# KAIST-VICLab/MoBGS

Measured on AMD Instinct MI355X. Metric: train-step renders/sec (fwd+bwd, 1352x1014, 300k Gaussians), higher is better.
Workload: dtype f32; 1 GPU; BASELINE config #2: seesaw-synth (SURVEY 8d seed 0), 200000 static + 100000 dynamic Gaussians, 1352x1014, render() lean mode fwd+bwd incl. spline prep, decoder, camera gradient; gaussians=300000, visible=287203, pixels=1370928, parallelism=single

## Files before the change

### mobgs_amd/csrc/decoder_shared.h

```cpp
#pragma once
#include "common.h"
#include "wave_shared.h"

namespace mobgs {

constexpr int W1_ROWS_SHARED = 2;

typedef const float __attribute__((address_space(4))) * ConstWeights;
__device__ __forceinline__ ConstWeights reload_here(const float* p) {
    unsigned long long v = (unsigned long long)p;
    asm volatile("" : "+s"(v));
    const unsigned lo = __builtin_amdgcn_readfirstlane((unsigned)v);
    const unsigned hi = __builtin_amdgcn_readfirstlane((unsigned)(v >> 32));
    return (ConstWeights)(((unsigned long long)hi << 32) | lo);
}

struct RayCam {
    float fx, fy, cx, cy;
    float c2w[12];
};
__device__ inline RayCam load_raycam(const float* __restrict__ intr, const float* __restrict__ c2w) {
    RayCam c;
    c.fx = intr[0]; c.fy = intr[1]; c.cx = intr[2]; c.cy = intr[3];
#pragma unroll
// ... 140 lines not shown
    vf[9] = g / ac;
    v_alpha = alpha > 1e-10f ? -g * f[9] / (ac * ac) : 0.f;
#pragma unroll
    for (int i = 0; i < 3; ++i) {
        vorg[i] = vx[6 + i];
        vdir[i] = vx[9 + i];
    }
}

struct WgradFinish {
    const float* w_partial = nullptr;
    float *g_w1 = nullptr, *g_w2 = nullptr, *g_c2w = nullptr;
    int rows_per_image = 0, n_images = 0, accumulate = 0, c2w_floats = 0;
};
constexpr int WGRAD_NRED = 102;
__host__ __device__ inline int wgrad_finish_outputs(const WgradFinish& f) {
    return WGRAD_NRED + ((f.g_c2w && f.c2w_floats == 16) ? 4 : 0);
}
__device__ inline void wgrad_column_sum(const WgradFinish& f, int k, int img) {
    float* g_c2w = f.g_c2w ? f.g_c2w + (size_t)img * f.c2w_floats : nullptr;
    if (k >= WGRAD_NRED) {
        if (threadIdx.x == 0) g_c2w[k - 90] = 0.f;
        return;
    }
    int first = 0, count = f.rows_per_image * f.n_images;
    if (k >= 90) {
        first = img * f.rows_per_image;
        count = f.rows_per_image;
    } else if (img != 0) {
        return;
    }
    const float* wp = f.w_partial + (size_t)first * WGRAD_NRED;
    float s = 0.f;
    for (int b = threadIdx.x; b < count; b += 256) s += wp[(size_t)b * WGRAD_NRED + k];
    MOBGS_WAVE_FOLD(s, MOBGS_WAVE_ADD);
    __shared__ float wgrad_red[4];
    if ((threadIdx.x & 63) == 0) wgrad_red[threadIdx.x >> 6] = s;
    __syncthreads();
    if (threadIdx.x == 0) {
        const float t = wgrad_red[0] + wgrad_red[1] + wgrad_red[2] + wgrad_red[3];
        if (k < 72)
            f.g_w1[k] = f.accumulate ? f.g_w1[k] + t : t;
        else if (k < 90)
            f.g_w2[k - 72] = f.accumulate ? f.g_w2[k - 72] + t : t;
        else if (g_c2w)
            g_c2w[k - 90] = t;
    }
}

size_t decoder_wgrad_scratch_floats(int C, int rows_per_image);
unsigned* decoder_wgrad_ticket(float* scratch, int C, int rows_per_image);
void launch_decoder_wgrad_reduce(int C, int rows_per_image, float* scratch, float* g_w1, float* g_w2, float* g_c2w,
                                 int g_c2w_floats, int accumulate, hipStream_t st);

}
```

### mobgs_amd/csrc/prep_shared.h

```cpp
#pragma once
#include <hip/hip_fp16.h>

#include "common.h"

namespace mobgs {

__device__ inline float ldf(const float* p, size_t i) { return p[i]; }
__device__ inline float ldf(const __half* p, size_t i) { return __half2float(p[i]); }
__device__ inline float4 ld4(const float* p, size_t i) { return reinterpret_cast<const float4*>(p)[i]; }
__device__ inline float4 ld4(const __half* p, size_t i) {
    const uint2 u = reinterpret_cast<const uint2*>(p)[i];
    const __half2 a = *reinterpret_cast<const __half2*>(&u.x), b = *reinterpret_cast<const __half2*>(&u.y);
    const float2 fa = __half22float2(a), fb = __half22float2(b);
    return make_float4(fa.x, fa.y, fb.x, fb.y);
}
__device__ inline void stf(float* p, size_t i, float v) { p[i] = v; }
__device__ inline void stf(__half* p, size_t i, float v) { p[i] = __float2half(v); }
__device__ inline void st4(float* p, size_t i, float4 v) { reinterpret_cast<float4*>(p)[i] = v; }
__device__ inline void st4(__half* p, size_t i, float4 v) {
    const __half2 a = __floats2half2_rn(v.x, v.y), b = __floats2half2_rn(v.z, v.w);
    uint2 u;
    u.x = *reinterpret_cast<const unsigned*>(&a);
    u.y = *reinterpret_cast<const unsigned*>(&b);
    reinterpret_cast<uint2*>(p)[i] = u;
// ... 58 lines not shown
            s[k] = expf(ldf(in.s_scaling, 3 * (size_t)i + k));
            col[6 + k] = 0.0f * ldf(in.s_ft, 3 * (size_t)i + k);
        }
        const float4 r = ld4(in.s_rotation, i);
        q[0] = r.x; q[1] = r.y; q[2] = r.z; q[3] = r.w;
        o = 1.f / (1.f + expf(-ldf(in.s_opacity, i)));
#pragma unroll
        for (int k = 0; k < 6; ++k) col[k] = ldf(in.s_fdc, 6 * (size_t)i + k);
    } else {
        const int j = i - in.Ns;
        const float t_feat = in.times[0], t_curve = in.times[1];
        const float tfp = t_feat - in.d_trbf[j];
        const int n = (int)in.d_ncp[j];
        const Hermite H = hermite_setup(t_curve, n);
        const float* cp = in.d_control + (size_t)j * 36;
#pragma unroll
        for (int k = 0; k < 3; ++k) {
            const float p0 = cp[3 * H.i0 + k], p1 = cp[3 * H.i1 + k], p2 = cp[3 * H.i2 + k], p3 = cp[3 * H.i3 + k];
            const float m0 = H.left_edge ? (p2 - p1) : (p2 - p0) * 0.5f;
            const float m1 = H.right_edge ? (p2 - p1) : (p3 - p1) * 0.5f;
            m[k] = (H.h00 * p1 + H.h10 * m0 + H.h01 * p2 + H.h11 * m1) * 1e-2f;
            s[k] = expf(ldf(in.d_scaling, 3 * (size_t)j + k));
            col[6 + k] = tfp * ldf(in.d_ft, 3 * (size_t)j + k);
        }
        const float4 r = ld4(in.d_rotation, j);
        const float4 w = ld4(in.d_omega, j);
        q[0] = r.x + tfp * w.x; q[1] = r.y + tfp * w.y; q[2] = r.z + tfp * w.z; q[3] = r.w + tfp * w.w;
        o = 1.f / (1.f + expf(-ldf(in.d_opacity, j)));
#pragma unroll
        for (int k = 0; k < 6; ++k) col[k] = ldf(in.d_fdc, 6 * (size_t)j + k);
    }
}

template <bool ACC, typename G>
__device__ __forceinline__ void prep_bwd_apply(
    int i, int Ns, const float* __restrict__ times, const long long* __restrict__ d_ncp,
    const float* __restrict__ d_trbf, const float (&vm)[3], const float (&vq)[4], const float (&vs)[3], float vo,
    const float (&vc)[9], float* __restrict__ g_s_xyz, G* __restrict__ g_s_scaling, G* __restrict__ g_s_rotation,
    G* __restrict__ g_s_opacity, G* __restrict__ g_s_fdc, G* __restrict__ g_s_ft, float* __restrict__ g_d_control,
    G* __restrict__ g_d_scaling, G* __restrict__ g_d_rotation, G* __restrict__ g_d_omega, G* __restrict__ g_d_opacity,
    G* __restrict__ g_d_fdc, G* __restrict__ g_d_ft) {
#pragma clang fp contract(off)
    if (i < Ns) {
#pragma unroll
        for (int k = 0; k < 3; ++k) {
            g_s_xyz[3 * i + k] = (ACC ? g_s_xyz[3 * i + k] : 0.f) + vm[k];
            stf(g_s_scaling, 3 * (size_t)i + k, (ACC ? ldf(g_s_scaling, 3 * (size_t)i + k) : 0.f) + vs[k]);
            stf(g_s_ft, 3 * (size_t)i + k, (ACC ? ldf(g_s_ft, 3 * (size_t)i + k) : 0.f) + 0.0f * vc[6 + k]);
        }
        {
            float4 q = make_float4(vq[0], vq[1], vq[2], vq[3]);
            if (ACC) {
                const float4 o = ld4(g_s_rotation, i);
                q = make_float4(o.x + q.x, o.y + q.y, o.z + q.z, o.w + q.w);
            }
            st4(g_s_rotation, i, q);
        }
        stf(g_s_opacity, i, (ACC ? ldf(g_s_opacity, i) : 0.f) + vo);
#pragma unroll
        for (int k = 0; k < 6; ++k) stf(g_s_fdc, 6 * (size_t)i + k, (ACC ? ldf(g_s_fdc, 6 * (size_t)i + k) : 0.f) + vc[k]);
    } else {
        const int j = i - Ns;
        const float tfp = times[0] - d_trbf[j];
        const int n = (int)d_ncp[j];
        const Hermite H = hermite_setup(times[1], n);
        float* gc = g_d_control + (size_t)j * 36;
#pragma unroll
        for (int k = 0; k < 3; ++k) {
            const float v = vm[k] * 1e-2f;
            float a0 = 0.f, a1 = H.h00 * v, a2 = H.h01 * v, a3 = 0.f;
            const float vm0 = H.h10 * v, vm1 = H.h11 * v;
            if (H.left_edge) {
                a2 += vm0;
                a1 -= vm0;
            } else {
                a2 += 0.5f * vm0;
                a0 -= 0.5f * vm0;
            }
            if (H.right_edge) {
                a2 += vm1;
                a1 -= vm1;
            } else {
                a3 += 0.5f * vm1;
                a1 -= 0.5f * vm1;
            }
            if (ACC) {
                if (!H.left_edge) gc[3 * H.i0 + k] += a0;
                gc[3 * H.i1 + k] += a1;
                gc[3 * H.i2 + k] += a2;
                if (!H.right_edge) gc[3 * H.i3 + k] += a3;
            } else {
                if (!H.left_edge) gc[3 * H.i0 + k] = a0;
                gc[3 * H.i1 + k] = a1;
                gc[3 * H.i2 + k] = a2;
                if (!H.right_edge) gc[3 * H.i3 + k] = a3;
            }
            stf(g_d_scaling, 3 * (size_t)j + k, (ACC ? ldf(g_d_scaling, 3 * (size_t)j + k) : 0.f) + vs[k]);
            stf(g_d_ft, 3 * (size_t)j + k, (ACC ? ldf(g_d_ft, 3 * (size_t)j + k) : 0.f) + tfp * vc[6 + k]);
        }
        {
            float4 q = make_float4(vq[0], vq[1], vq[2], vq[3]);
            float4 w = make_float4(tfp * vq[0], tfp * vq[1], tfp * vq[2], tfp * vq[3]);
            if (ACC) {
                const float4 o = ld4(g_d_rotation, j);
                const float4 p = ld4(g_d_omega, j);
                q = make_float4(o.x + q.x, o.y + q.y, o.z + q.z, o.w + q.w);
                w = make_float4(p.x + w.x, p.y + w.y, p.z + w.z, p.w + w.w);
            }
            st4(g_d_rotation, j, q);
            st4(g_d_omega, j, w);
        }
        stf(g_d_opacity, j, (ACC ? ldf(g_d_opacity, j) : 0.f) + vo);
#pragma unroll
        for (int k = 0; k < 6; ++k) stf(g_d_fdc, 6 * (size_t)j + k, (ACC ? ldf(g_d_fdc, 6 * (size_t)j + k) : 0.f) + vc[k]);
    }
}

__device__ __forceinline__ void prep_bwd_clear_rows(int Ns, int Nd, float* __restrict__ g_d_control) {
    const int wave_first = (blockIdx.x * blockDim.x + (threadIdx.x & ~63)) - Ns;
    const int j0 = max(wave_first, 0), j1 = min(wave_first + 64, Nd);
    if (j1 > j0) {
        float4* row = reinterpret_cast<float4*>(g_d_control + (size_t)j0 * 36);
        const int n4 = (j1 - j0) * 9;
        for (int t = threadIdx.x & 63; t < n4; t += 64) row[t] = make_float4(0.f, 0.f, 0.f, 0.f);
        __builtin_amdgcn_fence(__ATOMIC_RELEASE, "wavefront");
        __builtin_amdgcn_s_waitcnt(0);
    }
}

}
```

### mobgs_amd/csrc/project.hip

```cpp
#include <stdarg.h>

#include "isect_launch.h"
#include "prep_shared.h"
#include "wave_shared.h"

namespace mobgs {

static thread_local char g_err[512] = "";
void set_error(const char* fmt, ...) {
    va_list ap;
    va_start(ap, fmt);
    vsnprintf(g_err, sizeof(g_err), fmt, ap);
    va_end(ap);
}

struct Cam {
    float R[9];
    float t[3];
    float fx, fy, cx, cy;
};

__device__ inline Cam load_cam(const float* __restrict__ viewmats, const float* __restrict__ Ks, int c) {
    Cam cam;
    const float* V = viewmats + 16 * c;
// ... 214 lines not shown
struct PrepBwdFused {
    int Ns, Nd, accumulate;
    const float* times;
    const long long* d_ncp;
    const float *d_trbf, *opac, *v_opac, *v_colors;
    const float *x_means, *x_quats, *x_scales;
    LeafGrads g;
};
template <bool PREPB>
__global__ void __launch_bounds__(256)
project_bwd_kernel(int N, const float* __restrict__ means, const float* __restrict__ quats,
                   const float* __restrict__ scales, const float* __restrict__ viewmats,
                   const float* __restrict__ Ks, int width, int height, float eps2d,
                   const int32_t* __restrict__ radii, const float* __restrict__ conics,
                   const float* __restrict__ v_means2d, const float* __restrict__ v_depths,
                   const float* __restrict__ v_conics, float* __restrict__ v_means,
                   float* __restrict__ v_quats, float* __restrict__ v_scales,
                   float* __restrict__ v_view_partial, int accumulate, int accumulate_scales, size_t geom_stride,
                   size_t scales_stride, PrepBwdFused pb) {
    const int i = blockIdx.x * blockDim.x + threadIdx.x;
    const int c = blockIdx.y;
    if constexpr (PREPB) {
        if (!pb.accumulate) prep_bwd_clear_rows(pb.Ns, pb.Nd, pb.g.d_control);
    }
    means += 3 * c * geom_stride;
    quats += 4 * c * geom_stride;
    v_means += 3 * c * geom_stride;
    v_quats += 4 * c * geom_stride;
    v_scales += 3 * c * scales_stride;
    const Cam cam = load_cam(viewmats, Ks, c);
    float vR[9] = {0.f, 0.f, 0.f, 0.f, 0.f, 0.f, 0.f, 0.f, 0.f};
    float vt[3] = {0.f, 0.f, 0.f};
    float vm[3] = {0.f, 0.f, 0.f}, vq[4] = {0.f, 0.f, 0.f, 0.f}, vs[3] = {0.f, 0.f, 0.f};
    const size_t o = (size_t)c * N + (i < N ? i : 0);
    const bool live = (i < N) && radii[o] > 0;
    if (live) {
        const float m[3] = {means[3 * i], means[3 * i + 1], means[3 * i + 2]};
        float p[3];
#pragma unroll
        for (int r = 0; r < 3; ++r)
            p[r] = cam.R[3 * r] * m[0] + cam.R[3 * r + 1] * m[1] + cam.R[3 * r + 2] * m[2] + cam.t[r];
        const float4 qv = reinterpret_cast<const float4*>(quats)[i];
        const float qraw[4] = {qv.x, qv.y, qv.z, qv.w};
        const float s[3] = {scales[3 * i], scales[3 * i + 1], scales[3 * i + 2]};
        float Rq[9], M[9], S3[9], RS[9], Sc[9];
        quat_to_rotmat(qraw, Rq);
#pragma unroll
        for (int r = 0; r < 3; ++r) {
            M[3 * r] = Rq[3 * r] * s[0];
            M[3 * r + 1] = Rq[3 * r + 1] * s[1];
            M[3 * r + 2] = Rq[3 * r + 2] * s[2];
        }
        mm3_abt(M, M, S3);
        mm3(cam.R, S3, RS);
        mm3_abt(RS, cam.R, Sc);
        const Persp P = persp_setup(cam, p, width, height);

        const float X0 = conics[3 * o], X1 = conics[3 * o + 1], X2 = conics[3 * o + 2];
        float g0 = 0.f, g1 = 0.f, g2 = 0.f;
        if (v_conics) {
            g0 = v_conics[3 * o];
            g1 = 0.5f * v_conics[3 * o + 1];
            g2 = v_conics[3 * o + 2];
        }
        const float A00 = X0 * g0 + X1 * g1, A01 = X0 * g1 + X1 * g2;
        const float A10 = X1 * g0 + X2 * g1, A11 = X1 * g1 + X2 * g2;
        const float vS00 = -(A00 * X0 + A01 * X1), vS01 = -(A00 * X1 + A01 * X2);
        const float vS10 = -(A10 * X0 + A11 * X1), vS11 = -(A10 * X1 + A11 * X2);

        float vSJ[6];
#pragma unroll
        for (int k = 0; k < 3; ++k) {
            vSJ[k] = vS00 * P.J[k] + vS01 * P.J[3 + k];
            vSJ[3 + k] = vS10 * P.J[k] + vS11 * P.J[3 + k];
        }
        float vSc[9];
#pragma unroll
        for (int a = 0; a < 3; ++a)
#pragma unroll
            for (int b = 0; b < 3; ++b) vSc[3 * a + b] = P.J[a] * vSJ[b] + P.J[3 + a] * vSJ[3 + b];
        float vStJ[6];
#pragma unroll
        for (int k = 0; k < 3; ++k) {
            vStJ[k] = vS00 * P.J[k] + vS10 * P.J[3 + k];
            vStJ[3 + k] = vS01 * P.J[k] + vS11 * P.J[3 + k];
        }
        float vJ[6];
#pragma unroll
        for (int r = 0; r < 2; ++r)
#pragma unroll
            for (int k = 0; k < 3; ++k) {
                vJ[3 * r + k] = vSJ[3 * r] * Sc[3 * k] + vSJ[3 * r + 1] * Sc[3 * k + 1] + vSJ[3 * r + 2] * Sc[3 * k + 2] +
                                vStJ[3 * r] * Sc[k] + vStJ[3 * r + 1] * Sc[3 + k] + vStJ[3 * r + 2] * Sc[6 + k];
            }

        float vp[3] = {0.f, 0.f, 0.f};
        float gx = 0.f, gy = 0.f;
        if (v_means2d) {
            gx = v_means2d[2 * o];
            gy = v_means2d[2 * o + 1];
        }
        const float rz = P.rz, rz2 = P.rz2, rz3 = rz2 * rz;
        vp[0] += cam.fx * rz * gx;
        vp[1] += cam.fy * rz * gy;
        vp[2] += -(cam.fx * p[0] * gx + cam.fy * p[1] * gy) * rz2;
        const float xr = p[0] * rz, yr = p[1] * rz;
        if (xr <= P.lim_x_pos && xr >= -P.lim_x_neg)
            vp[0] += -cam.fx * rz2 * vJ[2];
        else
            vp[2] += -cam.fx * rz3 * vJ[2] * P.tx;
        if (yr <= P.lim_y_pos && yr >= -P.lim_y_neg)
            vp[1] += -cam.fy * rz2 * vJ[5];
        else
            vp[2] += -cam.fy * rz3 * vJ[5] * P.ty;
        vp[2] += -cam.fx * rz2 * vJ[0] - cam.fy * rz2 * vJ[4] + 2.f * cam.fx * P.tx * rz3 * vJ[2] +
                 2.f * cam.fy * P.ty * rz3 * vJ[5];
        if (v_depths) vp[2] += v_depths[o];

#pragma unroll
        for (int r = 0; r < 3; ++r) {
            vt[r] = vp[r];
#pragma unroll
            for (int k = 0; k < 3; ++k) vR[3 * r + k] = vp[r] * m[k];
        }
#pragma unroll
        for (int k = 0; k < 3; ++k) vm[k] = cam.R[k] * vp[0] + cam.R[3 + k] * vp[1] + cam.R[6 + k] * vp[2];

        float RS3t[9];
        mm3_abt(cam.R, S3, RS3t);
        float T1[9], T2[9];
        mm3(vSc, RS3t, T1);
        mm3_atb(vSc, RS, T2);
#pragma unroll
        for (int k = 0; k < 9; ++k) vR[k] += T1[k] + T2[k];
        float RtV[9], vS3[9];
        mm3_atb(cam.R, vSc, RtV);
        mm3(RtV, cam.R, vS3);

        float Sy[9], vM[9];
#pragma unroll
        for (int a = 0; a < 3; ++a)
#pragma unroll
            for (int b = 0; b < 3; ++b) Sy[3 * a + b] = vS3[3 * a + b] + vS3[3 * b + a];
        mm3(Sy, M, vM);
        float vRq[9];
#pragma unroll
        for (int r = 0; r < 3; ++r)
#pragma unroll
            for (int k = 0; k < 3; ++k) vRq[3 * r + k] = vM[3 * r + k] * s[k];
#pragma unroll
        for (int k = 0; k < 3; ++k) vs[k] = Rq[k] * vM[k] + Rq[3 + k] * vM[3 + k] + Rq[6 + k] * vM[6 + k];
        const float inv = 1.f / sqrtf(qraw[1] * qraw[1] + qraw[2] * qraw[2] + qraw[3] * qraw[3] + qraw[0] * qraw[0]);
        const float w = qraw[0] * inv, x = qraw[1] * inv, y = qraw[2] * inv, z = qraw[3] * inv;
        float vn[4];
        vn[0] = 2.f * (-z * vRq[1] + y * vRq[2] + z * vRq[3] - x * vRq[5] - y * vRq[6] + x * vRq[7]);
        vn[1] = 2.f * (y * vRq[1] + z * vRq[2] + y * vRq[3] - 2.f * x * vRq[4] - w * vRq[5] + z * vRq[6] + w * vRq[7] -
                       2.f * x * vRq[8]);
        vn[2] = 2.f * (-2.f * y * vRq[0] + x * vRq[1] + w * vRq[2] + x * vRq[3] + z * vRq[5] - w * vRq[6] + z * vRq[7] -
                       2.f * y * vRq[8]);
        vn[3] = 2.f * (-2.f * z * vRq[0] - w * vRq[1] + x * vRq[2] + w * vRq[3] - 2.f * z * vRq[4] + y * vRq[5] +
                       x * vRq[6] + y * vRq[7]);
        const float dotp = vn[0] * w + vn[1] * x + vn[2] * y + vn[3] * z;
        vq[0] = (vn[0] - dotp * w) * inv;
        vq[1] = (vn[1] - dotp * x) * inv;
        vq[2] = (vn[2] - dotp * y) * inv;
        vq[3] = (vn[3] - dotp * z) * inv;
    }
    if constexpr (PREPB) {
        if (i < N) {
            float vsx[3], vo = 0.f, vc[9];
#pragma unroll
            for (int k = 0; k < 9; ++k) vc[k] = pb.v_colors ? pb.v_colors[9 * i + k] : 0.f;
#pragma unroll
            for (int k = 0; k < 3; ++k) {
                if (pb.x_means) vm[k] = vm[k] + pb.x_means[3 * i + k];
                const float t = pb.x_scales ? vs[k] + pb.x_scales[3 * i + k] : vs[k];
                vsx[k] = t * scales[3 * i + k];
            }
            if (pb.x_quats) {
                const float4 r = reinterpret_cast<const float4*>(pb.x_quats)[i];
                vq[0] = vq[0] + r.x; vq[1] = vq[1] + r.y; vq[2] = vq[2] + r.z; vq[3] = vq[3] + r.w;
            }
            if (pb.v_opac) {
                const float op = pb.opac[i];
                vo = pb.v_opac[i] * op * (1.f - op);
            }
            const LeafGrads& g = pb.g;
            if (pb.accumulate)
                prep_bwd_apply<true, float>(i, pb.Ns, pb.times, pb.d_ncp, pb.d_trbf, vm, vq, vsx, vo, vc, g.s_xyz,
                                            g.s_scaling, g.s_rotation, g.s_opacity, g.s_fdc, g.s_ft, g.d_control,
                                            g.d_scaling, g.d_rotation, g.d_omega, g.d_opacity, g.d_fdc, g.d_ft);
            else
                prep_bwd_apply<false, float>(i, pb.Ns, pb.times, pb.d_ncp, pb.d_trbf, vm, vq, vsx, vo, vc, g.s_xyz,
                                             g.s_scaling, g.s_rotation, g.s_opacity, g.s_fdc, g.s_ft, g.d_control,
                                             g.d_scaling, g.d_rotation, g.d_omega, g.d_opacity, g.d_fdc, g.d_ft);
        }
    } else if (i < N) {
        if (accumulate) {
            v_means[3 * i] += vm[0];
            v_means[3 * i + 1] += vm[1];
            v_means[3 * i + 2] += vm[2];
            float4 a = reinterpret_cast<float4*>(v_quats)[i];
            a.x += vq[0];
            a.y += vq[1];
            a.z += vq[2];
            a.w += vq[3];
            reinterpret_cast<float4*>(v_quats)[i] = a;
        } else {
            v_means[3 * i] = vm[0];
            v_means[3 * i + 1] = vm[1];
            v_means[3 * i + 2] = vm[2];
            reinterpret_cast<float4*>(v_quats)[i] = make_float4(vq[0], vq[1], vq[2], vq[3]);
        }
        if (accumulate_scales) {
            v_scales[3 * i] += vs[0];
            v_scales[3 * i + 1] += vs[1];
            v_scales[3 * i + 2] += vs[2];
        } else {
            v_scales[3 * i] = vs[0];
            v_scales[3 * i + 1] = vs[1];
            v_scales[3 * i + 2] = vs[2];
        }
    }
    if constexpr (PREPB) {
        if (!v_view_partial) return;
    }
    __shared__ float red[4][12];
    const int lane = threadIdx.x & 63, wv = threadIdx.x >> 6;
// ... 197 lines not shown
```

### mobgs_amd/csrc/raster.hip

```cpp
#include <tuple>
#include <type_traits>

#include "common.h"
#include "decoder_shared.h"
#include "raster_launch.h"
#include "raster_shared.h"

namespace mobgs {

__global__ void __launch_bounds__(256)
pack_records_kernel(int N, int channels, int stride, const float* __restrict__ means2d,
                    const float* __restrict__ conics, const float* __restrict__ colors, int colors_per_camera,
                    const float* __restrict__ opacities, int opac_per_camera, const float* __restrict__ extra,
                    const int32_t* __restrict__ radii, float* __restrict__ records) {
    const int i = blockIdx.x * blockDim.x + threadIdx.x;
    const int c = blockIdx.y;
    if (i >= N) return;
    const size_t o = (size_t)c * N + i;
    if (radii[o] <= 0) return;
    const float2 m = reinterpret_cast<const float2*>(means2d)[o];
    write_splat_record(records + o * stride, m.x, m.y, conics[3 * o], conics[3 * o + 1], conics[3 * o + 2],
                       opacities[opac_per_camera ? o : (size_t)i], colors + (colors_per_camera ? o : (size_t)i) * channels,
                       channels, extra != nullptr, extra ? extra[o] : 0.f);
}
// ... 1394 lines not shown
        s1.x += u1.x; s1.y += u1.y; s1.z += u1.z; s1.w += u1.w;
        s2.x += u2.x; s2.y += u2.y; s2.z += u2.z; s2.w += u2.w;
        s3.x += u3.x; s3.y += u3.y; s3.z += u3.z; s3.w += u3.w;
    }
    for (; k < b; ++k) {
        const float4 u = p[(size_t)k * rq];
        s0.x += u.x; s0.y += u.y; s0.z += u.z; s0.w += u.w;
    }
    float acc[4] = {(s0.x + s1.x) + (s2.x + s3.x), (s0.y + s1.y) + (s2.y + s3.y), (s0.z + s1.z) + (s2.z + s3.z),
                    (s0.w + s1.w) + (s2.w + s3.w)};
    const size_t g = (size_t)gid;
    if (q == 0)
        finish_geometry(records + g * 4 * rq, b > a, acc[0], acc[1], acc[2]);
    else if (q == 1) {
        acc[0] *= 0.5f;
        acc[1] = (b > a && acc[1] != 0.f) ? -acc[1] * __builtin_amdgcn_exp2f(-records[g * 4 * rq + 5]) : 0.f;
    }
#pragma unroll
    for (int i = 0; i < 4; ++i) {
        const int comp = 4 * q + i;
        if (comp < 2)
            v_means2d[2 * g + comp] = acc[i];
        else if (comp < 5)
            v_conics[3 * g + (comp - 2)] = acc[i];
        else if (comp == 5)
            v_opacities[g] = acc[i];
        else if (comp - 6 < channels)
            v_colors[g * channels + (comp - 6)] = acc[i];
        else if (has_extra && comp - 6 == channels)
            v_extra[g] = acc[i];
    }
}

template <int LPS, bool WRED = false>
__global__ void __launch_bounds__(256)
slot_reduce16_kernel(int n_gauss, int channels, int has_extra, const int32_t* __restrict__ cum_tiles,
                     const int32_t* __restrict__ keep_scan, const float* __restrict__ grad_slots,
                     float* __restrict__ v_means2d, float* __restrict__ v_conics, float* __restrict__ v_opacities,
                     float* __restrict__ v_colors, float* __restrict__ v_extra,
                     const int32_t* __restrict__ any_record, const float* __restrict__ records,
                     const int32_t* __restrict__ tiles_per_gauss, WgradFinish wf = WgradFinish{}) {
    constexpr int SUBS = LPS / 4;
    int bid = blockIdx.x;
    if constexpr (WRED) {
        const int nout = wgrad_finish_outputs(wf), nw = nout * wf.n_images;
        if (bid < nw) {
            wgrad_column_sum(wf, bid % nout, bid / nout);
            return;
        }
        bid -= nw;
    }
    const int gid = (bid * blockDim.x + threadIdx.x) / LPS;
    const int l16 = threadIdx.x & (LPS - 1);
    const int q = l16 & 3, sub = l16 >> 2;
    const bool live = gid < n_gauss;
    int a = 0, b = 0;
    if (live && !(any_record && *any_record == 0)) {
        a = keep_index(keep_scan, cum_tiles[gid]);
        b = keep_index(keep_scan, box_end(cum_tiles, tiles_per_gauss, gid));
    }
    float4 s0 = make_float4(0.f, 0.f, 0.f, 0.f), s1 = s0;
    const float4* p = reinterpret_cast<const float4*>(grad_slots) + q;
    int k = a + sub;
    for (; k + SUBS < b; k += 2 * SUBS) {
        const float4 u = p[(size_t)k * 4], v = p[(size_t)(k + SUBS) * 4];
        s0.x += u.x; s0.y += u.y; s0.z += u.z; s0.w += u.w;
        s1.x += v.x; s1.y += v.y; s1.z += v.z; s1.w += v.w;
    }
    if (k < b) {
        const float4 u = p[(size_t)k * 4];
        s0.x += u.x; s0.y += u.y; s0.z += u.z; s0.w += u.w;
    }
    float acc[4] = {s0.x + s1.x, s0.y + s1.y, s0.z + s1.z, s0.w + s1.w};
#pragma unroll
    for (int i = 0; i < 4; ++i) {
        if (SUBS == 4) {
            acc[i] = dpp_add<0x124>(acc[i]);
            acc[i] = dpp_add<0x128>(acc[i]);
        } else if (SUBS == 2) {
            acc[i] = dpp_add_xor4(acc[i]);
        }
    }
    if (!live || sub != 0) return;
    const size_t g = (size_t)gid;
    if (q == 0)
        finish_geometry(records + g * 16, b > a, acc[0], acc[1], acc[2]);
    else if (q == 1) {
        acc[0] *= 0.5f;
        acc[1] = (b > a && acc[1] != 0.f) ? -acc[1] * __builtin_amdgcn_exp2f(-records[g * 16 + 5]) : 0.f;
    }
#pragma unroll
    for (int i = 0; i < 4; ++i) {
        const int comp = 4 * q + i;
        const float v = acc[i];
        if (comp < 2)
            v_means2d[2 * g + comp] = v;
        else if (comp < 5)
            v_conics[3 * g + (comp - 2)] = v;
        else if (comp == 5)
            v_opacities[g] = v;
        else if (comp - 6 < channels)
            v_colors[g * channels + (comp - 6)] = v;
        else if (has_extra && comp - 6 == channels)
            v_extra[g] = v;
    }
}

struct SplatInputs {
    const float *means2d, *conics, *colors, *opacities, *extra;
    const int32_t* radii;
    int colors_per_camera, opac_per_camera;
};
static void launch_pack(int C, int N, int channels, const SplatInputs& in, float* records, hipStream_t st) {
    hipLaunchKernelGGL(pack_records_kernel, dim3((N + 255) / 256, C), dim3(256), 0, st, N, channels,
                       record_stride(channels + (in.extra ? 1 : 0)), in.means2d, in.conics, in.colors, in.colors_per_camera,
                       in.opacities, in.opac_per_camera, in.extra, in.radii, records);
}

}

using namespace mobgs;


extern "C" {

int mobgs_cotangent_probe(int n_arrays, const float* const* arrays, const size_t* counts, int32_t* live, void* stream) {
    hipStream_t st = (hipStream_t)stream;
    if (n_arrays < 0 || !live || (n_arrays > 0 && (!arrays || !counts))) {
        set_error("mobgs_cotangent_probe: bad arguments");
        return MOBGS_E_INVALID;
    }
    (void)hipMemsetAsync(live, 0, sizeof(int32_t), st);
    for (int a0 = 0; a0 < n_arrays; a0 += PROBE_MAX) {
        ProbeTable t;
        int m = 0;
        size_t longest = 0;
        for (int a = a0; a < n_arrays && a < a0 + PROBE_MAX; ++a) {
            if (!arrays[a] || counts[a] == 0) continue;
            t.p[m] = arrays[a];
// ... 187 lines not shown
        return MOBGS_E_INVALID;
    }
    if (C > 1 && g_c2w && c2w_stride == 0) {
        set_error("mobgs_raster_bwd_decode_finish: a pose shared by the images of a batch cannot receive a gradient");
        return MOBGS_E_INVALID;
    }
    launch_decoder_wgrad_reduce(C, tiles_per_image(width, height), w_partial, g_w1, g_w2, g_c2w, g_c2w_floats,
                                accumulate_wgrad, (hipStream_t)stream);
    return check_launch("decoder_wgrad_reduce_rows_kernel");
}

int mobgs_raster_bwd_reduce_decode(int C, int N, const float* records, const int32_t* cum_tiles, const int32_t* keep_scan,
                                   const float* grad_slots, const int32_t* any_record, float* v_means2d, float* v_conics,
                                   float* v_opacities, float* v_colors, float* v_extra, const int32_t* tiles_per_gauss,
                                   int width, int height, const float* w_partial, int c2w_stride, float* g_w1, float* g_w2,
                                   float* g_c2w, int g_c2w_floats, int accumulate_wgrad, void* stream) {
    if (C <= 0 || N < 0 || width <= 0 || height <= 0 || ((long long)C * N > 0 && !records) || !w_partial || !g_w1 || !g_w2 ||
        (g_c2w && g_c2w_floats != 12 && g_c2w_floats != 16) || (C > 1 && g_c2w && c2w_stride == 0)) {
        set_error("mobgs_raster_bwd_reduce_decode: bad arguments (w_partial, g_w1, g_w2 required; g_c2w: 12 or 16 floats per "
                  "image, one pose per image)");
        return MOBGS_E_INVALID;
    }
    WgradFinish wf;
    wf.w_partial = w_partial;
    wf.g_w1 = g_w1;
    wf.g_w2 = g_w2;
    wf.g_c2w = g_c2w;
    wf.rows_per_image = tiles_per_image(width, height);
    wf.n_images = C;
    wf.accumulate = accumulate_wgrad;
    wf.c2w_floats = g_c2w_floats;
    const int n = C * N;
    const int extra = wgrad_finish_outputs(wf) * C;
    hipLaunchKernelGGL((slot_reduce16_kernel<8, true>), dim3(extra + (int)(((size_t)n * 8 + 255) / 256)), dim3(256), 0,
                       (hipStream_t)stream, n, 9, 1, cum_tiles, keep_scan, grad_slots, v_means2d, v_conics, v_opacities,
                       v_colors, v_extra, any_record, records, tiles_per_gauss, wf);
    return check_launch("slot_reduce16_kernel(+wgrad)");
}

size_t mobgs_raster_bwd_decode_scratch_floats(int C, int width, int height) {
    if (C <= 0 || width <= 0 || height <= 0) return 0;
    return decoder_wgrad_scratch_floats(C, tiles_per_image(width, height));
}

int mobgs_raster_class_fwd(int C, int N, int Ns, int class_sel, int channels_total, int width, int height,
                           const float* records, const float* backgrounds, const int32_t* tile_offsets,
                           const int32_t* tile_order, const int32_t* flatten_ids, float* render, float* alphas,
                           int32_t* last_ids, uint8_t* isect_reach, const MobgsTuning* tuning, void* stream) {
    if (C <= 0 || N <= 0 || Ns < 0 || Ns > N || (class_sel != 1 && class_sel != 2) ||
        (channels_total != 10 && channels_total != 1)) {
        set_error("mobgs_raster_class_fwd: unsupported arguments (C=%d N=%d Ns=%d class=%d D=%d)", C, N, Ns, class_sel,
                  channels_total);
        return MOBGS_E_UNSUPPORTED;
    }
    const RasterGrid g = raster_grid(C, width, height, tile_order, TILES_PER_WG);
    const RasterFwdArgs a{records, backgrounds, tile_offsets, tile_order, flatten_ids, render, alphas, last_ids, isect_reach};
    const ClassSel cls{class_sel, N, Ns, tuning_all_reach(tuning)};
    hipStream_t st = (hipStream_t)stream;
    if (raster_plan(channels_total, 1, g.nt, tuning).fwd_blocks)
        launch_raster_fwd(raster_fwd_blocks_kernel<10, true>, g, a, st, cls, DecodeEpi{});
    else if (channels_total == 10)
        launch_raster_fwd(raster_fwd_kernel<10, true>, g, a, st, cls);
    else
        launch_raster_fwd(raster_fwd_kernel<1, true>, g, a, st, cls);
    return check_launch("raster_fwd_kernel(class)");
}

// ... 16 lines not shown
    ClassSel cls{class_sel, N, Ns, tuning_all_reach(tuning)};
    cls.static_rows = tuning_static_rows(tuning);
    cls.set_n = N;
    if (plan.gate)
        cls.gate = arm_cotangent_gate(tuning, v_render, (size_t)C * height * width * channels_total, v_alphas,
                                      (size_t)C * height * width, any_record, st);
    if (plan.mfma()) {
        const int rc = raster_bwd_mfma_launch(plan.bwd, channels_total, true, g, a, cls, st);
        return rc != MOBGS_OK ? rc : check_launch("raster_bwd_mfma_kernel(class)");
    }
    if (channels_total == 10)
        launch_raster_bwd(raster_bwd_kernel<10, true>, g, a, st, cls, DecodeBwd{});
    else
        launch_raster_bwd(raster_bwd_kernel<1, true>, g, a, st, cls, DecodeBwd{});
    return check_launch("raster_bwd_kernel(class)");
}

int mobgs_raster_bwd_reduce(int C, int N, int channels, int has_extra, const float* records,
                            const int32_t* cum_tiles, const int32_t* keep_scan, const float* grad_slots,
                            const int32_t* any_record, float* v_means2d, float* v_conics, float* v_opacities,
                            float* v_colors, float* v_extra, const int32_t* tiles_per_gauss, void* stream) {
    hipStream_t st = (hipStream_t)stream;
    const int D = channels + (has_extra ? 1 : 0);
    const int stride = record_stride(D);
    if (stride > 32) {
        set_error("mobgs_raster_bwd_reduce: %d total channels not compiled in (at most 26: records of 32 floats)", D);
        return MOBGS_E_UNSUPPORTED;
    }
    if (C <= 0 || N < 0 || D < 1 || ((long long)C * N > 0 && !records)) {
        set_error("mobgs_raster_bwd_reduce: bad sizes C=%d N=%d channels=%d", C, N, channels);
        return MOBGS_E_INVALID;
    }
    const int n = C * N;
    auto launch = [&](auto kernel, int lanes, auto lead, auto tail) {
        std::apply([&](auto... args) {
            hipLaunchKernelGGL(kernel, dim3((int)(((size_t)n * lanes + 255) / 256)), dim3(256), 0, st, n, channels,
                               has_extra, args...);
        }, std::tuple_cat(lead, std::make_tuple(cum_tiles, keep_scan, grad_slots, v_means2d, v_conics, v_opacities,
                                                v_colors, v_extra, any_record, records, tiles_per_gauss), tail));
    };
    const auto quarters = std::make_tuple(stride / 4);
    const std::tuple<> none;
    if (n > 0) {
        if (stride == 8)
            launch(slot_reduce_wide_kernel<2>, 2, quarters, none);
        else if (stride == 12)
            launch(slot_reduce_wide_kernel<4>, 4, quarters, none);
        else if (stride == 16)
            launch(slot_reduce16_kernel<8, false>, 8, none, std::make_tuple(WgradFinish{}));
        else
            launch(slot_reduce_wide_kernel<8>, 8, quarters, none);
    }
    return check_launch("slot_reduce kernels");
}

}
```

Before: 1154 renders/s.

## Make slot reduce persistent with software-prefetched row metadata and hoisted loads

Converts slot_reduce16_kernel into a persistent grid-stride kernel sized to about 8 workgroups per CU. It prefetches the next rows' tile spans, keep-scan entries and record heads one and two iterations ahead, and unrolls the slot accumulation four-wide. The projection backward kernel now issues all of its per-Gaussian loads (radii, means, quats, conic grads, prep-backward inputs) up front without branching, then masks results with the live flag. The wgrad column sum is also unrolled eight-wide. Together these aim to hide memory latency, at the cost of extra register pressure and some loads for dead Gaussians.

```diff
diff --git a/mobgs_amd/csrc/decoder_shared.h b/mobgs_amd/csrc/decoder_shared.h
--- a/mobgs_amd/csrc/decoder_shared.h
+++ b/mobgs_amd/csrc/decoder_shared.h
@@ -196,7 +196,13 @@
     }
     const float* wp = f.w_partial + (size_t)first * WGRAD_NRED;
     float s = 0.f;
-    for (int b = threadIdx.x; b < count; b += 256) s += wp[(size_t)b * WGRAD_NRED + k];
+    for (int b = threadIdx.x; b < count; b += 8 * 256) {
+        float x[8];
+#pragma unroll
+        for (int u = 0; u < 8; ++u) x[u] = wp[(size_t)min(b + u * 256, count - 1) * WGRAD_NRED + k];
+#pragma unroll
+        for (int u = 0; u < 8; ++u) s = (b + u * 256 < count) ? s + x[u] : s;
+    }
     MOBGS_WAVE_FOLD(s, MOBGS_WAVE_ADD);
     __shared__ float wgrad_red[4];
     if ((threadIdx.x & 63) == 0) wgrad_red[threadIdx.x >> 6] = s;
diff --git a/mobgs_amd/csrc/prep_shared.h b/mobgs_amd/csrc/prep_shared.h
--- a/mobgs_amd/csrc/prep_shared.h
+++ b/mobgs_amd/csrc/prep_shared.h
@@ -114,10 +114,13 @@
     }
 }
 
+struct PrepBwdRow {
+    float t_feat, t_curve, trbf;
+    int ncp;
+};
 template <bool ACC, typename G>
 __device__ __forceinline__ void prep_bwd_apply(
-    int i, int Ns, const float* __restrict__ times, const long long* __restrict__ d_ncp,
-    const float* __restrict__ d_trbf, const float (&vm)[3], const float (&vq)[4], const float (&vs)[3], float vo,
+    int i, int Ns, PrepBwdRow row, const float (&vm)[3], const float (&vq)[4], const float (&vs)[3], float vo,
     const float (&vc)[9], float* __restrict__ g_s_xyz, G* __restrict__ g_s_scaling, G* __restrict__ g_s_rotation,
     G* __restrict__ g_s_opacity, G* __restrict__ g_s_fdc, G* __restrict__ g_s_ft, float* __restrict__ g_d_control,
     G* __restrict__ g_d_scaling, G* __restrict__ g_d_rotation, G* __restrict__ g_d_omega, G* __restrict__ g_d_opacity,
@@ -143,9 +146,9 @@
         for (int k = 0; k < 6; ++k) stf(g_s_fdc, 6 * (size_t)i + k, (ACC ? ldf(g_s_fdc, 6 * (size_t)i + k) : 0.f) + vc[k]);
     } else {
         const int j = i - Ns;
-        const float tfp = times[0] - d_trbf[j];
-        const int n = (int)d_ncp[j];
-        const Hermite H = hermite_setup(times[1], n);
+        const float tfp = row.t_feat - row.trbf;
+        const int n = row.ncp;
+        const Hermite H = hermite_setup(row.t_curve, n);
         float* gc = g_d_control + (size_t)j * 36;
 #pragma unroll
         for (int k = 0; k < 3; ++k) {
@@ -197,6 +200,19 @@
         for (int k = 0; k < 6; ++k) stf(g_d_fdc, 6 * (size_t)j + k, (ACC ? ldf(g_d_fdc, 6 * (size_t)j + k) : 0.f) + vc[k]);
     }
 }
+template <bool ACC, typename G>
+__device__ __forceinline__ void prep_bwd_apply(
+    int i, int Ns, const float* __restrict__ times, const long long* __restrict__ d_ncp,
+    const float* __restrict__ d_trbf, const float (&vm)[3], const float (&vq)[4], const float (&vs)[3], float vo,
+    const float (&vc)[9], float* __restrict__ g_s_xyz, G* __restrict__ g_s_scaling, G* __restrict__ g_s_rotation,
+    G* __restrict__ g_s_opacity, G* __restrict__ g_s_fdc, G* __restrict__ g_s_ft, float* __restrict__ g_d_control,
+    G* __restrict__ g_d_scaling, G* __restrict__ g_d_rotation, G* __restrict__ g_d_omega, G* __restrict__ g_d_opacity,
+    G* __restrict__ g_d_fdc, G* __restrict__ g_d_ft) {
+    PrepBwdRow row{0.f, 0.f, 0.f, 0};
+    if (i >= Ns) row = PrepBwdRow{times[0], times[1], d_trbf[i - Ns], (int)d_ncp[i - Ns]};
+    prep_bwd_apply<ACC, G>(i, Ns, row, vm, vq, vs, vo, vc, g_s_xyz, g_s_scaling, g_s_rotation, g_s_opacity, g_s_fdc, g_s_ft,
+                           g_d_control, g_d_scaling, g_d_rotation, g_d_omega, g_d_opacity, g_d_fdc, g_d_ft);
+}
 
 __device__ __forceinline__ void prep_bwd_clear_rows(int Ns, int Nd, float* __restrict__ g_d_control) {
     const int wave_first = (blockIdx.x * blockDim.x + (threadIdx.x & ~63)) - Ns;
diff --git a/mobgs_amd/csrc/project.hip b/mobgs_amd/csrc/project.hip
--- a/mobgs_amd/csrc/project.hip
+++ b/mobgs_amd/csrc/project.hip
@@ -270,17 +270,58 @@
     float vR[9] = {0.f, 0.f, 0.f, 0.f, 0.f, 0.f, 0.f, 0.f, 0.f};
     float vt[3] = {0.f, 0.f, 0.f};
     float vm[3] = {0.f, 0.f, 0.f}, vq[4] = {0.f, 0.f, 0.f, 0.f}, vs[3] = {0.f, 0.f, 0.f};
-    const size_t o = (size_t)c * N + (i < N ? i : 0);
-    const bool live = (i < N) && radii[o] > 0;
-    if (live) {
-        const float m[3] = {means[3 * i], means[3 * i + 1], means[3 * i + 2]};
+    const int ic = min(i, N - 1);
+    const size_t o = (size_t)c * N + ic;
+    const int32_t rad = radii[o];
+    const float m[3] = {means[3 * ic], means[3 * ic + 1], means[3 * ic + 2]};
+    const float4 qv = reinterpret_cast<const float4*>(quats)[ic];
+    const float s[3] = {scales[3 * ic], scales[3 * ic + 1], scales[3 * ic + 2]};
+    const float X0 = conics[3 * o], X1 = conics[3 * o + 1], X2 = conics[3 * o + 2];
+    float g0 = 0.f, g1 = 0.f, g2 = 0.f, gx = 0.f, gy = 0.f, gz = 0.f;
+    if (v_conics) {
+        g0 = v_conics[3 * o];
+        g1 = v_conics[3 * o + 1];
+        g2 = v_conics[3 * o + 2];
+    }
+    if (v_means2d) {
+        gx = v_means2d[2 * o];
+        gy = v_means2d[2 * o + 1];
+    }
+    if (v_depths) gz = v_depths[o];
+    float vc[9] = {0.f, 0.f, 0.f, 0.f, 0.f, 0.f, 0.f, 0.f, 0.f}, xm[3] = {0.f, 0.f, 0.f}, xs[3] = {0.f, 0.f, 0.f};
+    float4 xq = make_float4(0.f, 0.f, 0.f, 0.f);
+    float op = 0.f, vop = 0.f;
+    PrepBwdRow prow{0.f, 0.f, 0.f, 0};
+    if constexpr (PREPB) {
+        if (pb.v_colors) {
+#pragma unroll
+            for (int k = 0; k < 9; ++k) vc[k] = pb.v_colors[9 * ic + k];
+        }
+        if (pb.x_means) {
+#pragma unroll
+            for (int k = 0; k < 3; ++k) xm[k] = pb.x_means[3 * ic + k];
+        }
+        if (pb.x_scales) {
+#pragma unroll
+            for (int k = 0; k < 3; ++k) xs[k] = pb.x_scales[3 * ic + k];
+        }
+        if (pb.x_quats) xq = reinterpret_cast<const float4*>(pb.x_quats)[ic];
+        if (pb.v_opac) {
+            op = pb.opac[ic];
+            vop = pb.v_opac[ic];
+        }
+        if (pb.Nd > 0) {
+            const int jc = max(ic - pb.Ns, 0);
+            prow = PrepBwdRow{pb.times[0], pb.times[1], pb.d_trbf[jc], (int)pb.d_ncp[jc]};
+        }
+    }
+    const bool live = (i < N) && rad > 0;
+    {
         float p[3];
 #pragma unroll
         for (int r = 0; r < 3; ++r)
             p[r] = cam.R[3 * r] * m[0] + cam.R[3 * r + 1] * m[1] + cam.R[3 * r + 2] * m[2] + cam.t[r];
-        const float4 qv = reinterpret_cast<const float4*>(quats)[i];
         const float qraw[4] = {qv.x, qv.y, qv.z, qv.w};
-        const float s[3] = {scales[3 * i], scales[3 * i + 1], scales[3 * i + 2]};
         float Rq[9], M[9], S3[9], RS[9], Sc[9];
         quat_to_rotmat(qraw, Rq);
 #pragma unroll
@@ -294,13 +335,7 @@
         mm3_abt(RS, cam.R, Sc);
         const Persp P = persp_setup(cam, p, width, height);
 
-        const float X0 = conics[3 * o], X1 = conics[3 * o + 1], X2 = conics[3 * o + 2];
-        float g0 = 0.f, g1 = 0.f, g2 = 0.f;
-        if (v_conics) {
-            g0 = v_conics[3 * o];
-            g1 = 0.5f * v_conics[3 * o + 1];
-            g2 = v_conics[3 * o + 2];
-        }
+        g1 = 0.5f * g1;
         const float A00 = X0 * g0 + X1 * g1, A01 = X0 * g1 + X1 * g2;
         const float A10 = X1 * g0 + X2 * g1, A11 = X1 * g1 + X2 * g2;
         const float vS00 = -(A00 * X0 + A01 * X1), vS01 = -(A00 * X1 + A01 * X2);
@@ -333,11 +368,6 @@
             }
 
         float vp[3] = {0.f, 0.f, 0.f};
-        float gx = 0.f, gy = 0.f;
-        if (v_means2d) {
-            gx = v_means2d[2 * o];
-            gy = v_means2d[2 * o + 1];
-        }
         const float rz = P.rz, rz2 = P.rz2, rz3 = rz2 * rz;
         vp[0] += cam.fx * rz * gx;
         vp[1] += cam.fy * rz * gy;
@@ -353,7 +383,7 @@
             vp[2] += -cam.fy * rz3 * vJ[5] * P.ty;
         vp[2] += -cam.fx * rz2 * vJ[0] - cam.fy * rz2 * vJ[4] + 2.f * cam.fx * P.tx * rz3 * vJ[2] +
                  2.f * cam.fy * P.ty * rz3 * vJ[5];
-        if (v_depths) vp[2] += v_depths[o];
+        if (v_depths) vp[2] += gz;
 
 #pragma unroll
         for (int r = 0; r < 3; ++r) {
@@ -404,34 +434,40 @@
         vq[2] = (vn[2] - dotp * y) * inv;
         vq[3] = (vn[3] - dotp * z) * inv;
     }
+#pragma unroll
+    for (int k = 0; k < 9; ++k) vR[k] = live ? vR[k] : 0.f;
+#pragma unroll
+    for (int k = 0; k < 3; ++k) {
+        vt[k] = live ? vt[k] : 0.f;
+        vm[k] = live ? vm[k] : 0.f;
+        vs[k] = live ? vs[k] : 0.f;
+    }
+#pragma unroll
+    for (int k = 0; k < 4; ++k) vq[k] = live ? vq[k] : 0.f;
     if constexpr (PREPB) {
+#pragma unroll
+        for (int k = 0; k < 9; ++k) vc[k] = live ? vc[k] : 0.f;
+        float vsx[3], vo = 0.f;
+#pragma unroll
+        for (int k = 0; k < 3; ++k) {
+            if (pb.x_means) vm[k] = vm[k] + xm[k];
+            const float t = pb.x_scales ? vs[k] + xs[k] : vs[k];
+            vsx[k] = t * s[k];
+        }
+        if (pb.x_quats) {
+            vq[0] = vq[0] + xq.x; vq[1] = vq[1] + xq.y; vq[2] = vq[2] + xq.z; vq[3] = vq[3] + xq.w;
+        }
+        if (pb.v_opac) vo = vop * op * (1.f - op);
         if (i < N) {
-            float vsx[3], vo = 0.f, vc[9];
-#pragma unroll
-            for (int k = 0; k < 9; ++k) vc[k] = pb.v_colors ? pb.v_colors[9 * i + k] : 0.f;
-#pragma unroll
-            for (int k = 0; k < 3; ++k) {
-                if (pb.x_means) vm[k] = vm[k] + pb.x_means[3 * i + k];
-                const float t = pb.x_scales ? vs[k] + pb.x_scales[3 * i + k] : vs[k];
-                vsx[k] = t * scales[3 * i + k];
-            }
-            if (pb.x_quats) {
-                const float4 r = reinterpret_cast<const float4*>(pb.x_quats)[i];
-                vq[0] = vq[0] + r.x; vq[1] = vq[1] + r.y; vq[2] = vq[2] + r.z; vq[3] = vq[3] + r.w;
-            }
-            if (pb.v_opac) {
-                const float op = pb.opac[i];
-                vo = pb.v_opac[i] * op * (1.f - op);
-            }
             const LeafGrads& g = pb.g;
             if (pb.accumulate)
-                prep_bwd_apply<true, float>(i, pb.Ns, pb.times, pb.d_ncp, pb.d_trbf, vm, vq, vsx, vo, vc, g.s_xyz,
-                                            g.s_scaling, g.s_rotation, g.s_opacity, g.s_fdc, g.s_ft, g.d_control,
-                                            g.d_scaling, g.d_rotation, g.d_omega, g.d_opacity, g.d_fdc, g.d_ft);
+                prep_bwd_apply<true, float>(i, pb.Ns, prow, vm, vq, vsx, vo, vc, g.s_xyz, g.s_scaling, g.s_rotation,
+                                            g.s_opacity, g.s_fdc, g.s_ft, g.d_control, g.d_scaling, g.d_rotation,
+                                            g.d_omega, g.d_opacity, g.d_fdc, g.d_ft);
             else
-                prep_bwd_apply<false, float>(i, pb.Ns, pb.times, pb.d_ncp, pb.d_trbf, vm, vq, vsx, vo, vc, g.s_xyz,
-                                             g.s_scaling, g.s_rotation, g.s_opacity, g.s_fdc, g.s_ft, g.d_control,
-                                             g.d_scaling, g.d_rotation, g.d_omega, g.d_opacity, g.d_fdc, g.d_ft);
+                prep_bwd_apply<false, float>(i, pb.Ns, prow, vm, vq, vsx, vo, vc, g.s_xyz, g.s_scaling, g.s_rotation,
+                                             g.s_opacity, g.s_fdc, g.s_ft, g.d_control, g.d_scaling, g.d_rotation,
+                                             g.d_omega, g.d_opacity, g.d_fdc, g.d_ft);
         }
     } else if (i < N) {
         if (accumulate) {
diff --git a/mobgs_amd/csrc/raster.hip b/mobgs_amd/csrc/raster.hip
--- a/mobgs_amd/csrc/raster.hip
+++ b/mobgs_amd/csrc/raster.hip
@@ -1450,63 +1450,33 @@
     }
 }
 
-template <int LPS, bool WRED = false>
-__global__ void __launch_bounds__(256)
-slot_reduce16_kernel(int n_gauss, int channels, int has_extra, const int32_t* __restrict__ cum_tiles,
-                     const int32_t* __restrict__ keep_scan, const float* __restrict__ grad_slots,
-                     float* __restrict__ v_means2d, float* __restrict__ v_conics, float* __restrict__ v_opacities,
-                     float* __restrict__ v_colors, float* __restrict__ v_extra,
-                     const int32_t* __restrict__ any_record, const float* __restrict__ records,
-                     const int32_t* __restrict__ tiles_per_gauss, WgradFinish wf = WgradFinish{}) {
-    constexpr int SUBS = LPS / 4;
-    int bid = blockIdx.x;
-    if constexpr (WRED) {
-        const int nout = wgrad_finish_outputs(wf), nw = nout * wf.n_images;
-        if (bid < nw) {
-            wgrad_column_sum(wf, bid % nout, bid / nout);
-            return;
-        }
-        bid -= nw;
-    }
-    const int gid = (bid * blockDim.x + threadIdx.x) / LPS;
-    const int l16 = threadIdx.x & (LPS - 1);
-    const int q = l16 & 3, sub = l16 >> 2;
-    const bool live = gid < n_gauss;
-    int a = 0, b = 0;
-    if (live && !(any_record && *any_record == 0)) {
-        a = keep_index(keep_scan, cum_tiles[gid]);
-        b = keep_index(keep_scan, box_end(cum_tiles, tiles_per_gauss, gid));
-    }
-    float4 s0 = make_float4(0.f, 0.f, 0.f, 0.f), s1 = s0;
-    const float4* p = reinterpret_cast<const float4*>(grad_slots) + q;
-    int k = a + sub;
-    for (; k + SUBS < b; k += 2 * SUBS) {
-        const float4 u = p[(size_t)k * 4], v = p[(size_t)(k + SUBS) * 4];
-        s0.x += u.x; s0.y += u.y; s0.z += u.z; s0.w += u.w;
-        s1.x += v.x; s1.y += v.y; s1.z += v.z; s1.w += v.w;
-    }
-    if (k < b) {
-        const float4 u = p[(size_t)k * 4];
-        s0.x += u.x; s0.y += u.y; s0.z += u.z; s0.w += u.w;
-    }
-    float acc[4] = {s0.x + s1.x, s0.y + s1.y, s0.z + s1.z, s0.w + s1.w};
-#pragma unroll
-    for (int i = 0; i < 4; ++i) {
-        if (SUBS == 4) {
-            acc[i] = dpp_add<0x124>(acc[i]);
-            acc[i] = dpp_add<0x128>(acc[i]);
-        } else if (SUBS == 2) {
-            acc[i] = dpp_add_xor4(acc[i]);
-        }
-    }
-    if (!live || sub != 0) return;
-    const size_t g = (size_t)gid;
-    if (q == 0)
-        finish_geometry(records + g * 16, b > a, acc[0], acc[1], acc[2]);
-    else if (q == 1) {
-        acc[0] *= 0.5f;
-        acc[1] = (b > a && acc[1] != 0.f) ? -acc[1] * __builtin_amdgcn_exp2f(-records[g * 16 + 5]) : 0.f;
-    }
+constexpr int SLOT_REDUCE_WG_PER_CU = 8;
+struct SlotRowSpan { int32_t start, other; };
+struct SlotRowKeep { int32_t a0, a1, b0, b1; };
+struct SlotRowHead { float2 lo, hi; };
+__device__ __forceinline__ SlotRowSpan slot_row_span(const int32_t* __restrict__ cum_tiles,
+                                                     const int32_t* __restrict__ tiles_per_gauss, int g) {
+    const int32_t* other = tiles_per_gauss ? tiles_per_gauss + g : cum_tiles + g + 1;
+    return {cum_tiles[g], *other};
+}
+__device__ __forceinline__ SlotRowKeep slot_row_keep(const int32_t* __restrict__ keep_scan, SlotRowSpan s, bool counts) {
+    const int end = counts ? s.start + s.other : s.other;
+    const int32_t* pa = keep_scan + (size_t)(s.start >> KEEP_CHUNK_LOG2) * (KEEP_CHUNK + 1);
+    const int32_t* pb = keep_scan + (size_t)(end >> KEEP_CHUNK_LOG2) * (KEEP_CHUNK + 1);
+    return {pa[0], pa[1 + (s.start & (KEEP_CHUNK - 1))], pb[0], pb[1 + (end & (KEEP_CHUNK - 1))]};
+}
+__device__ __forceinline__ SlotRowHead slot_row_head(const float* __restrict__ records, int g) {
+    const float2* r = reinterpret_cast<const float2*>(records + (size_t)g * 16);
+    return {r[1], r[2]};
+}
+__device__ __forceinline__ void slot_row_arrived(const SlotRowSpan& s, const SlotRowKeep& k, const SlotRowHead& h) {
+    asm volatile("" ::"v"(s.start), "v"(s.other), "v"(k.a0), "v"(k.a1), "v"(k.b0), "v"(k.b1), "v"(h.lo.x), "v"(h.lo.y),
+                 "v"(h.hi.x), "v"(h.hi.y));
+}
+__device__ __forceinline__ void slot_row_store(size_t g, int q, const float (&acc)[4], int channels, int has_extra,
+                                               float* __restrict__ v_means2d, float* __restrict__ v_conics,
+                                               float* __restrict__ v_opacities, float* __restrict__ v_colors,
+                                               float* __restrict__ v_extra) {
 #pragma unroll
     for (int i = 0; i < 4; ++i) {
         const int comp = 4 * q + i;
@@ -1523,6 +1493,116 @@
             v_extra[g] = v;
     }
 }
+template <int LPS, bool WRED = false>
+__attribute__((amdgpu_waves_per_eu(8)))
+__global__ void __launch_bounds__(256)
+slot_reduce16_kernel(int n_gauss, int channels, int has_extra, const int32_t* __restrict__ cum_tiles,
+                     const int32_t* __restrict__ keep_scan, const float* __restrict__ grad_slots,
+                     float* __restrict__ v_means2d, float* __restrict__ v_conics, float* __restrict__ v_opacities,
+                     float* __restrict__ v_colors, float* __restrict__ v_extra,
+                     const int32_t* __restrict__ any_record, const float* __restrict__ records,
+                     const int32_t* __restrict__ tiles_per_gauss, WgradFinish wf = WgradFinish{}) {
+    constexpr int SUBS = LPS / 4;
+    int bid = blockIdx.x, row_wgs = gridDim.x;
+    if constexpr (WRED) {
+        const int nout = wgrad_finish_outputs(wf), nw = nout * wf.n_images;
+        if (bid < nw) {
+            wgrad_column_sum(wf, bid % nout, bid / nout);
+            return;
+        }
+        bid -= nw;
+        row_wgs -= nw;
+    }
+    const int G = row_wgs * (256 / LPS);
+    int g = (bid * blockDim.x + threadIdx.x) / LPS;
+    const int l16 = threadIdx.x & (LPS - 1);
+    const int q = l16 & 3, sub = l16 >> 2;
+    if (g >= n_gauss) return;
+    const int last = n_gauss - 1;
+    if (any_record && *any_record == 0) {
+        const float zero[4] = {0.f, 0.f, 0.f, 0.f};
+        if (sub == 0)
+            for (; g <= last; g += G)
+                slot_row_store((size_t)g, q, zero, channels, has_extra, v_means2d, v_conics, v_opacities, v_colors, v_extra);
+        return;
+    }
+    const float4* p = reinterpret_cast<const float4*>(grad_slots) + q;
+    const bool counts = tiles_per_gauss != nullptr;
+    SlotRowSpan span1 = slot_row_span(cum_tiles, tiles_per_gauss, min(g + G, last));
+    SlotRowKeep keep0 = slot_row_keep(keep_scan, slot_row_span(cum_tiles, tiles_per_gauss, g), counts);
+    SlotRowHead head0 = slot_row_head(records, g);
+    slot_row_arrived(span1, keep0, head0);
+    for (;;) {
+        const int g1 = min(g + G, last);
+        const SlotRowSpan span2 = slot_row_span(cum_tiles, tiles_per_gauss, min(g1 + G, last));
+        const SlotRowKeep keep1 = slot_row_keep(keep_scan, span1, counts);
+        const SlotRowHead head1 = slot_row_head(records, g1);
+        const int a = keep0.a0 + keep0.a1, b = keep0.b0 + keep0.b1;
+        float4 s0 = make_float4(0.f, 0.f, 0.f, 0.f), s1 = s0;
+        int k = a + sub;
+        const float4* pk = p + (size_t)k * 4;
+        for (; k + 3 * SUBS < b; k += 4 * SUBS, pk += 16 * SUBS) {
+            const float4 u0 = pk[0], v0 = pk[4 * SUBS], u1 = pk[8 * SUBS], v1 = pk[12 * SUBS];
+            s0.x += u0.x; s0.y += u0.y; s0.z += u0.z; s0.w += u0.w;
+            s1.x += v0.x; s1.y += v0.y; s1.z += v0.z; s1.w += v0.w;
+            s0.x += u1.x; s0.y += u1.y; s0.z += u1.z; s0.w += u1.w;
+            s1.x += v1.x; s1.y += v1.y; s1.z += v1.z; s1.w += v1.w;
+        }
+        if (k + SUBS < b) {
+            const float4 u = pk[0], v = pk[4 * SUBS];
+            s0.x += u.x; s0.y += u.y; s0.z += u.z; s0.w += u.w;
+            s1.x += v.x; s1.y += v.y; s1.z += v.z; s1.w += v.w;
+            k += 2 * SUBS;
+            pk += 8 * SUBS;
+        }
+        if (k < b) {
+            const float4 u = pk[0];
+            s0.x += u.x; s0.y += u.y; s0.z += u.z; s0.w += u.w;
+        }
+        slot_row_arrived(span2, keep1, head1);
+        float acc[4] = {s0.x + s1.x, s0.y + s1.y, s0.z + s1.z, s0.w + s1.w};
+#pragma unroll
+        for (int i = 0; i < 4; ++i) {
+            if (SUBS == 4) {
+                acc[i] = dpp_add<0x124>(acc[i]);
+                acc[i] = dpp_add<0x128>(acc[i]);
+            } else if (SUBS == 2) {
+                acc[i] = dpp_add_xor4(acc[i]);
+            }
+        }
+        if (sub == 0) {
+            if (q == 0) {
+                const float rec[6] = {0.f, 0.f, head0.lo.x, head0.lo.y, head0.hi.x, head0.hi.y};
+                finish_geometry(rec, b > a, acc[0], acc[1], acc[2]);
+            } else if (q == 1) {
+                acc[0] *= 0.5f;
+                acc[1] = (b > a && acc[1] != 0.f) ? -acc[1] * __builtin_amdgcn_exp2f(-head0.hi.y) : 0.f;
+            }
+            int qs = q;
+            asm volatile("" : "+v"(qs));
+            slot_row_store((size_t)g, qs, acc, channels, has_extra, v_means2d, v_conics, v_opacities, v_colors, v_extra);
+        }
+        if (g + G > last) break;
+        g = g1;
+        span1 = span2;
+        keep0 = keep1;
+        head0 = head1;
+    }
+}
+static int slot_reduce_workgroups(int n, int lanes, int lead = 0) {
+    static int cus[64] = {};
+    int dev = 0;
+    (void)hipGetDevice(&dev);
+    const int slot = (unsigned)dev < 64u ? dev : 0;
+    if (cus[slot] <= 0 || slot != dev) {
+        int v = 0;
+        if (hipDeviceGetAttribute(&v, hipDeviceAttributeMultiprocessorCount, dev) != hipSuccess || v <= 0) v = 256;
+        cus[slot] = v;
+    }
+    const size_t one_per_row = ((size_t)n * lanes + 255) / 256;
+    const int resident = std::max(SLOT_REDUCE_WG_PER_CU * cus[slot] - lead, cus[slot]);
+    return (int)std::min<size_t>(one_per_row, (size_t)resident);
+}
 
 struct SplatInputs {
     const float *means2d, *conics, *colors, *opacities, *extra;
@@ -1776,7 +1856,7 @@
     wf.c2w_floats = g_c2w_floats;
     const int n = C * N;
     const int extra = wgrad_finish_outputs(wf) * C;
-    hipLaunchKernelGGL((slot_reduce16_kernel<8, true>), dim3(extra + (int)(((size_t)n * 8 + 255) / 256)), dim3(256), 0,
+    hipLaunchKernelGGL((slot_reduce16_kernel<8, true>), dim3(extra + slot_reduce_workgroups(n, 8, extra)), dim3(256), 0,
                        (hipStream_t)stream, n, 9, 1, cum_tiles, keep_scan, grad_slots, v_means2d, v_conics, v_opacities,
                        v_colors, v_extra, any_record, records, tiles_per_gauss, wf);
     return check_launch("slot_reduce16_kernel(+wgrad)");
@@ -1859,24 +1939,24 @@
         return MOBGS_E_INVALID;
     }
     const int n = C * N;
-    auto launch = [&](auto kernel, int lanes, auto lead, auto tail) {
+    auto launch = [&](auto kernel, int wgs, auto lead, auto tail) {
         std::apply([&](auto... args) {
-            hipLaunchKernelGGL(kernel, dim3((int)(((size_t)n * lanes + 255) / 256)), dim3(256), 0, st, n, channels,
-                               has_extra, args...);
+            hipLaunchKernelGGL(kernel, dim3(wgs), dim3(256), 0, st, n, channels, has_extra, args...);
         }, std::tuple_cat(lead, std::make_tuple(cum_tiles, keep_scan, grad_slots, v_means2d, v_conics, v_opacities,
                                                 v_colors, v_extra, any_record, records, tiles_per_gauss), tail));
     };
+    auto one_per_row = [&](int lanes) { return (int)(((size_t)n * lanes + 255) / 256); };
     const auto quarters = std::make_tuple(stride / 4);
     const std::tuple<> none;
     if (n > 0) {
         if (stride == 8)
-            launch(slot_reduce_wide_kernel<2>, 2, quarters, none);
+            launch(slot_reduce_wide_kernel<2>, one_per_row(2), quarters, none);
         else if (stride == 12)
-            launch(slot_reduce_wide_kernel<4>, 4, quarters, none);
+            launch(slot_reduce_wide_kernel<4>, one_per_row(4), quarters, none);
         else if (stride == 16)
-            launch(slot_reduce16_kernel<8, false>, 8, none, std::make_tuple(WgradFinish{}));
+            launch(slot_reduce16_kernel<8, false>, slot_reduce_workgroups(n, 8), none, std::make_tuple(WgradFinish{}));
         else
-            launch(slot_reduce_wide_kernel<8>, 8, quarters, none);
+            launch(slot_reduce_wide_kernel<8>, one_per_row(8), quarters, none);
     }
     return check_launch("slot_reduce kernels");
 }
```

Result: no change. 1163 renders/s, median of 6 (+0.8%).
